# olivier-2018/scene_3Dreconstruction_MVSNet

Measured on AMD Instinct MI355X. Metric: depth maps/sec at N=5 views, 640x512, D=192; achieved HBM GB/s, higher is better.
Workload: dtype f32 (conv0, conv2-4, conv9, conv11: 3xbf16 split operands on the bf16 matrix cores, fp32 accumulate)

## Files before the change

scene_3dreconstruction_mvsnet_amd/csrc/conv0_split.hip:

```cpp
#include <cstdlib>
#include <cstring>
#include <type_traits>

#include "mvs_internal.h"
#include "storage.h"

#ifndef MVS_ABLATE
#define MVS_ABLATE 0
#endif

namespace mvs {

namespace c43s {
constexpr int TZ = 4, TY = 4, TX = 32;
constexpr int HY = TY + 2, HX = TX + 2;
constexpr int NT_PLANES = 6;
constexpr int VOX = HY * HX;
constexpr int PLANE_E = VOX * 8;
constexpr int PIECE_E = NT_PLANES * PLANE_E;
constexpr int TILE_E = 3 * PIECE_E;
constexpr int NCOL = VOX * 2;
constexpr int CPT = (NCOL + 255) / 256;
constexpr int NPOS = TY * TX;
constexpr int EXS = 12;
constexpr int BFRAG = 4 * NT_PLANES * 3 * 3;
static_assert(NT_PLANES * NPOS * EXS * 4 <= TILE_E * 2, "exchange tile must fit in the input tile");
}

typedef unsigned int su32x4 __attribute__((ext_vector_type(4)));
typedef unsigned int su32x2 __attribute__((ext_vector_type(2)));
typedef __bf16 sbf16x8 __attribute__((ext_vector_type(8)));
typedef __bf16 sbf16x4 __attribute__((ext_vector_type(4)));

__device__ __forceinline__ void split3(const f32x4 v, su32x2& p1, su32x2& p2, su32x2& p3) {
    const sbf16x4 h1 = __builtin_convertvector(v, sbf16x4);
    const f32x4 r1 = v - __builtin_convertvector(h1, f32x4);
    const sbf16x4 h2 = __builtin_convertvector(r1, sbf16x4);
    const f32x4 r2 = r1 - __builtin_convertvector(h2, f32x4);
    const sbf16x4 h3 = __builtin_convertvector(r2, sbf16x4);
    p1 = __builtin_bit_cast(su32x2, h1);
    p2 = __builtin_bit_cast(su32x2, h2);
    p3 = __builtin_bit_cast(su32x2, h3);
}

__device__ __forceinline__ f32x4 mfma_bf16(su32x4 a, su32x4 b, f32x4 c) {
    return __builtin_amdgcn_mfma_f32_16x16x32_bf16(__builtin_bit_cast(sbf16x8, a), __builtin_bit_cast(sbf16x8, b), c, 0, 0, 0);
}

template <int PAR>
__device__ __forceinline__ void c43s_chunk_mfmas(const unsigned short* __restrict__ tile, const int (&aoff)[3],
                                                 const su32x4 (&B)[2][3][3], f32x4 (&acc)[3][2]) {
    using namespace c43s;
#pragma unroll
    for (int p = 0; p < 3; ++p) {
        su32x4 a[3][4];
#pragma unroll
        for (int i = 0; i < 3; ++i)
#pragma unroll
            for (int j = 0; j < 4; ++j)
                a[i][j] = *reinterpret_cast<const su32x4*>(tile + p * PIECE_E + aoff[i] + j * HX * 8);
#pragma unroll
        for (int ky = 0; ky < 3; ++ky)
#pragma unroll
            for (int q = 0; q < 3 - p; ++q)
#pragma unroll
                for (int i = 0; i < 3; ++i) {
                    const int pl = i == 0 ? 0 : (i == 2 ? 1 : PAR);
#pragma unroll
                    for (int rr = 0; rr < 2; ++rr)
                        acc[i][rr] = mfma_bf16(a[i][rr + ky], B[pl][ky][q], acc[i][rr]);
                }
    }
}

__global__ __launch_bounds__(256, 2) void conv0_w43s_kernel(
    const float* __restrict__ x,
    const unsigned short* __restrict__ bp,
    const float* __restrict__ bias,
    float* __restrict__ y,
    int D, int H, int W
#if MVS_ABLATE == 50
    , long long* __restrict__ dbg
#endif
    ) {
    using namespace c43s;
#if MVS_ABLATE == 50
#define MVS_TICK(slot) if (dbg && blockIdx.x == 2000 && (threadIdx.x & 63) == 0) dbg[(threadIdx.x >> 6) * 32 + (slot)] = clock64();
#else
#define MVS_TICK(slot)
#endif
    __shared__ __attribute__((aligned(16))) unsigned short tile[TILE_E];

    const int tid = threadIdx.x, lane = tid & 63, wave = tid >> 6;
    const int nbx = (W + TX - 1) / TX, nby = (H + TY - 1) / TY;
    int bx, by, bz;
    if (nby % 8 == 0 && gridDim.x % 8 == 0) {
        const int xcd = blockIdx.x & 7, rows = nby >> 3;
        int i = blockIdx.x >> 3;
        bx = i % nbx; i /= nbx;
        by = xcd * rows + i % rows;
        bz = i / rows;
    } else {
        int b = blockIdx.x;
        bx = b % nbx; b /= nbx;
        by = b % nby;
        bz = b / nby;
    }
    const int x0 = bx * TX, y0 = by * TY, z0 = bz * TZ;
    const size_t HW8 = (size_t)H * W * 8, V8 = (size_t)D * HW8;

    unsigned boff[CPT][NT_PLANES];
    int loff[CPT];
#pragma unroll
    for (int i = 0; i < CPT; ++i) {
        const int col = tid + i * 256;
        const int half = col & 1, v = col >> 1;
        const int hx = v % HX, hy = v / HX;
        const int gy = y0 + hy - 1, gx = x0 + hx - 1;
        const bool ok = col < NCOL && gy >= 0 && gy < H && gx >= 0 && gx < W;
        loff[i] = col < NCOL ? v * 2 + half : -1;
#pragma unroll
        for (int q = 0; q < NT_PLANES; ++q) {
            const int gz = z0 - 1 + q;
            boff[i][q] = (ok && gz >= 0 && gz < D) ? (unsigned)(((size_t)gz * HW8 + ((size_t)gy * W + gx) * 8 + half * 4) * 4)
                                                   : 0x80000000u;
        }
    }
    f32x4 stg[CPT][NT_PLANES];
    auto load_chunk = [&](int c) {
        const __amdgpu_buffer_rsrc_t rs = __builtin_amdgcn_make_buffer_rsrc(
            const_cast<float*>(x + (size_t)c * V8), (short)0, (int)(V8 * 4), 0x00020000);
#pragma unroll
        for (int i = 0; i < CPT; ++i)
#pragma unroll
            for (int q = 0; q < NT_PLANES; ++q)
                stg[i][q] = __builtin_bit_cast(f32x4, __builtin_amdgcn_raw_buffer_load_b128(rs, (int)boff[i][q], 0, 0));
    };
    auto store_chunk = [&]() {
        su32x2* t8 = reinterpret_cast<su32x2*>(tile);
#pragma unroll
        for (int i = 0; i < CPT; ++i)
            if (loff[i] >= 0) {
                const f32x4(&d)[NT_PLANES] = stg[i];
                const f32x4 t1 = d[4] - 4.0f * d[2], t2 = d[3] - 4.0f * d[1];
                const f32x4 t3 = d[4] - d[2], t4 = 2.0f * (d[3] - d[1]);
                f32x4 u[NT_PLANES];
                u[0] = 4.0f * d[0] - 5.0f * d[2] + d[4];
                u[1] = t1 + t2;
                u[2] = t1 - t2;
                u[3] = t3 + t4;
                u[4] = t3 - t4;
                u[5] = 4.0f * d[1] - 5.0f * d[3] + d[5];
#pragma unroll
                for (int t = 0; t < NT_PLANES; ++t) {
                    su32x2 p1, p2, p3;
                    split3(u[t], p1, p2, p3);
                    su32x2* dst = t8 + t * (PLANE_E / 4) + loff[i];
                    dst[0] = p1;
                    dst[PIECE_E / 4] = p2;
                    dst[2 * (PIECE_E / 4)] = p3;
                }
            }
    };

    const int r = lane & 15, g = lane >> 4;
    const int u0 = 3 * wave, pA = u0 >> 1;
    int aoff[3];
#pragma unroll
    for (int i = 0; i < 3; ++i) {
        const int u = u0 + i, pl = u >> 1, mg = u & 1;
        aoff[i] = pl * PLANE_E + ((2 * mg) * HX + 2 * r + g) * 8;
    }
    su32x4 B[2][3][3];
    auto load_b = [&](int c) {
        const su32x4* bsrc = reinterpret_cast<const su32x4*>(bp) + (size_t)((c * NT_PLANES + pA) * 9) * 64 + lane;
#pragma unroll
        for (int pl = 0; pl < 2; ++pl)
#pragma unroll
            for (int ky = 0; ky < 3; ++ky)
#pragma unroll
                for (int q = 0; q < 3; ++q) B[pl][ky][q] = bsrc[((pl * 3 + ky) * 3 + q) * 64];
    };

    f32x4 acc[3][2];
#pragma unroll
    for (int i = 0; i < 3; ++i)
#pragma unroll
        for (int n = 0; n < 2; ++n) acc[i][n] = (f32x4){0.f, 0.f, 0.f, 0.f};

    MVS_TICK(0)
    load_chunk(0);
    load_b(0);
    store_chunk();
    MVS_TICK(1)
    __syncthreads();
    MVS_TICK(2)

#pragma unroll 1
    for (int c = 0; c < 4; ++c) {
        if (c < 3) load_chunk(c + 1);
        MVS_TICK(3 + 5 * c)
        if (wave & 1) c43s_chunk_mfmas<1>(tile, aoff, B, acc);
        else c43s_chunk_mfmas<0>(tile, aoff, B, acc);
        MVS_TICK(4 + 5 * c)
        if (c < 3) {
            load_b(c + 1);
            __syncthreads();
            MVS_TICK(5 + 5 * c)
            store_chunk();
            MVS_TICK(6 + 5 * c)
            __syncthreads();
            MVS_TICK(7 + 5 * c)
        }
    }

    __syncthreads();
    float* ex = reinterpret_cast<float*>(tile);
    {
        const int n = lane & 15, jj = n >> 3, co = n & 7;
#pragma unroll
        for (int i = 0; i < 3; ++i) {
            const int u = u0 + i, pl = u >> 1, mg = u & 1;
#pragma unroll
            for (int rr = 0; rr < 2; ++rr)
#pragma unroll
                for (int e = 0; e < 4; ++e)
                    ex[(pl * NPOS + (2 * mg + rr) * TX + 2 * (4 * g + e) + jj) * EXS + co] = acc[i][rr][e];
        }
    }
    __syncthreads();
    const int pos = tid >> 1, ch = tid & 1;
    const int gy = y0 + (pos >> 5), gx = x0 + (pos & 31);
    if (gy >= H || gx >= W) return;
    f32x4 M[NT_PLANES];
#pragma unroll
    for (int q = 0; q < NT_PLANES; ++q) M[q] = *reinterpret_cast<const f32x4*>(ex + (q * NPOS + pos) * EXS + ch * 4);
    const f32x4 bv = *reinterpret_cast<const f32x4*>(bias + ch * 4);
    const f32x4 zero = (f32x4){0.f, 0.f, 0.f, 0.f};
    const f32x4 s12 = M[1] + M[2], d12 = M[1] - M[2], s34 = M[3] + M[4], d34 = M[3] - M[4];
    f32x4 o[TZ];
    o[0] = (M[0] + s12) + s34;
    o[1] = d12 + 2.0f * d34;
    o[2] = s12 + 4.0f * s34;
    o[3] = (d12 + 8.0f * d34) + M[5];
#pragma unroll
    for (int q = 0; q < TZ; ++q) {
        if (z0 + q >= D) break;
        const f32x4 v = __builtin_elementwise_max(o[q] + bv, zero);
        *reinterpret_cast<f32x4*>(y + (((size_t)(z0 + q) * H + gy) * W + gx) * 8 + ch * 4) = v;
    }
    MVS_TICK(24)
#undef MVS_TICK
}

constexpr int c43p_MAXT = 512;
typedef float sf32x2 __attribute__((ext_vector_type(2)));
typedef __bf16 sbf16x2 __attribute__((ext_vector_type(2)));

__device__ __forceinline__ sf32x2 split_stage(const sf32x2 a, unsigned& packed) {
    const sbf16x2 h = __builtin_convertvector(a, sbf16x2);
    packed = __builtin_bit_cast(unsigned, h);
    const sf32x2 w = {__uint_as_float(packed << 16), __uint_as_float(packed & 0xFFFF0000u)};
    return a - w;
}
__device__ __forceinline__ void split3x(const f32x4 v, su32x2& p1, su32x2& p2, su32x2& p3) {
    unsigned a0, a1, b0, b1, c0, c1;
    const sf32x2 r0 = split_stage((sf32x2){v.x, v.y}, a0), r1 = split_stage((sf32x2){v.z, v.w}, a1);
    const sf32x2 q0 = split_stage(r0, b0), q1 = split_stage(r1, b1);
    c0 = __builtin_bit_cast(unsigned, __builtin_convertvector(q0, sbf16x2));
    c1 = __builtin_bit_cast(unsigned, __builtin_convertvector(q1, sbf16x2));
    p1 = (su32x2){a0, a1};
    p2 = (su32x2){b0, b1};
    p3 = (su32x2){c0, c1};
}

template <int PAR>
__device__ __forceinline__ void c43p_step_mfmas(const unsigned short* __restrict__ tile, const int (&aoff)[3],
                                                const su32x4 (&B)[2][3][3], su32x4 (&Bn)[2][3][3],
                                                __amdgpu_buffer_rsrc_t brs, unsigned bvoff, unsigned bnext,
                                                f32x4 (&acc)[3][2]) {
    using namespace c43s;
    constexpr int NC = 9;
    su32x4 a[3][4];
    auto request = [&](int n) {
        const int pn = n / 3, in = n % 3;
#pragma unroll
        for (int j = 0; j < 4; ++j)
            a[n % 3][j] = *reinterpret_cast<const su32x4*>(tile + pn * PIECE_E + aoff[in] + j * HX * 8);
    };
    request(0);
    request(1);
#pragma unroll
    for (int n = 0; n < NC; ++n) {
        const int p = n / 3, i = n % 3;
        if (n + 2 < NC) request(n + 2);
        {
            const int f0 = 2 * n, f1 = 2 * n + 1;
            Bn[f0 / 9][(f0 / 3) % 3][f0 % 3] = __builtin_bit_cast(su32x4, __builtin_amdgcn_raw_buffer_load_b128(
                brs, (int)bvoff, (int)(bnext + (unsigned)f0 * 1024u), 0));
            Bn[f1 / 9][(f1 / 3) % 3][f1 % 3] = __builtin_bit_cast(su32x4, __builtin_amdgcn_raw_buffer_load_b128(
                brs, (int)bvoff, (int)(bnext + (unsigned)f1 * 1024u), 0));
        }
        const int pl = i == 0 ? 0 : (i == 2 ? 1 : PAR);
#pragma unroll
        for (int ky = 0; ky < 3; ++ky)
#pragma unroll
            for (int q = 0; q < 3 - p; ++q)
#pragma unroll
                for (int rr = 0; rr < 2; ++rr)
                    acc[i][rr] = mfma_bf16(a[n % 3][rr + ky], B[pl][ky][q], acc[i][rr]);
#if MVS_ABLATE != 58
        __builtin_amdgcn_sched_barrier(0);
#endif
    }
}

__global__ __launch_bounds__(512) void conv0_w43p_kernel(
    const float* __restrict__ x,
    const unsigned short* __restrict__ bp,
    const float* __restrict__ bias,
    float* __restrict__ y,
    int D, int H, int W, int nb
#if MVS_ABLATE == 55
    , long long* __restrict__ dbg
#endif
    ) {
    using namespace c43s;
#if MVS_ABLATE == 55
#define MVS_PTICK(k, slot) if (dbg && blockIdx.x == 100 && (k) == 5 && (threadIdx.x & 63) == 0 && ((threadIdx.x >> 6) & 3) == 0) dbg[(threadIdx.x >> 8) * 64 + (slot)] = clock64();
#else
#define MVS_PTICK(k, slot)
#endif
    __shared__ __attribute__((aligned(16))) unsigned short buf[2 * TILE_E];
    __shared__ __attribute__((aligned(16))) float ex[NT_PLANES * NPOS * EXS];
    __shared__ int org[c43p_MAXT][4];

#if MVS_ABLATE == 75
    const int lane = threadIdx.x & 63, pw_ = threadIdx.x >> 6;
    const int wave = ((pw_ & 2) << 1) | ((pw_ & 4) >> 1) | (pw_ & 1), tid = wave * 64 + lane;
#else
    const int tid = threadIdx.x, lane = tid & 63, wave = tid >> 6;
#endif
    const bool consumer = __builtin_amdgcn_readfirstlane(wave) < 4;
    const int nbx = (W + TX - 1) / TX, nby = (H + TY - 1) / TY;
    const int G = gridDim.x;
    const int ntile = (nb - (int)blockIdx.x + G - 1) / G;
    const size_t HW8 = (size_t)H * W * 8, V8 = (size_t)D * HW8;
    auto origin = [&](int idx, int& x0, int& y0, int& z0) {
        int bx, by, bz;
        if (nby % 8 == 0 && G % 8 == 0) {
            const int xcd = idx & 7, rows = nby >> 3;
            int i = idx >> 3;
            bx = i % nbx; i /= nbx;
            by = xcd * rows + i % rows;
            bz = i / rows;
        } else {
            int b = idx;
            bx = b % nbx; b /= nbx;
            by = b % nby;
            bz = b / nby;
        }
        x0 = bx * TX; y0 = by * TY; z0 = bz * TZ;
    };

    for (int j = tid; j < ntile; j += 512) {
        int x0, y0, z0;
        origin((int)blockIdx.x + j * G, x0, y0, z0);
        org[j][0] = x0; org[j][1] = y0; org[j][2] = z0;
    }
    __syncthreads();
    const int ptid = tid & 255;
    unsigned boff[CPT][NT_PLANES];
    int loff[CPT];
    int chy[CPT], chx[CPT], crel[CPT];
#pragma unroll
    for (int i = 0; i < CPT; ++i) {
        const int col = min(ptid + i * 256, NCOL - 1);
        loff[i] = col;
        const int half = col & 1, v = col >> 1;
        chx[i] = v % HX - 1;
        chy[i] = v / HX - 1;
        crel[i] = (chy[i] * W + chx[i]) * 8 + half * 4;
    }
    auto set_tile = [&](int j) {
        const int x0 = org[j][0], y0 = org[j][1], z0 = org[j][2];
        const int hw8 = (int)HW8, tbase = (y0 * W + x0) * 8;
#pragma unroll
        for (int i = 0; i < CPT; ++i) {
            const int gy = y0 + chy[i], gx = x0 + chx[i];
            const bool ok = (unsigned)gy < (unsigned)H && (unsigned)gx < (unsigned)W;
            const int cb = tbase + crel[i];
#pragma unroll
            for (int q = 0; q < NT_PLANES; ++q) {
                const int gz = z0 - 1 + q;
                boff[i][q] = (ok && (unsigned)gz < (unsigned)D) ? (unsigned)(gz * hw8 + cb) * 4u
                                                                  : 0x80000000u;
            }
        }
    };
    f32x4 stg[2][CPT][NT_PLANES];
    auto issue_loads = [&](int c, f32x4 (&st)[CPT][NT_PLANES]) {
        const __amdgpu_buffer_rsrc_t rs = __builtin_amdgcn_make_buffer_rsrc(
            const_cast<float*>(x + (size_t)c * V8), (short)0, (int)(V8 * 4), 0x00020000);
#pragma unroll
        for (int i = 0; i < CPT; ++i)
#pragma unroll
            for (int q = 0; q < NT_PLANES; ++q)
                st[i][q] = __builtin_bit_cast(f32x4, __builtin_amdgcn_raw_buffer_load_b128(rs, (int)boff[i][q], 0, 0));
    };
    auto process = [&](auto set_tag, unsigned short* dstbuf, auto load_tag, int cn) {
        constexpr int SET = decltype(set_tag)::value;
        constexpr bool LOAD = decltype(load_tag)::value;
        su32x2* t8 = reinterpret_cast<su32x2*>(dstbuf);
        const __amdgpu_buffer_rsrc_t rs = __builtin_amdgcn_make_buffer_rsrc(
            const_cast<float*>(x + (size_t)cn * V8), (short)0, (int)(V8 * 4), 0x00020000);
#pragma unroll
        for (int i = 0; i < CPT; ++i) {
            f32x4 d[NT_PLANES];
#pragma unroll
            for (int q = 0; q < NT_PLANES; ++q) d[q] = stg[SET][i][q];
            const f32x4 t1 = d[4] - 4.0f * d[2], t2 = d[3] - 4.0f * d[1];
            const f32x4 t3 = d[4] - d[2], t4 = 2.0f * (d[3] - d[1]);
            f32x4 u[NT_PLANES];
            u[0] = 4.0f * d[0] - 5.0f * d[2] + d[4];
            u[1] = t1 + t2;
            u[2] = t1 - t2;
            u[3] = t3 + t4;
            u[4] = t3 - t4;
            u[5] = 4.0f * d[1] - 5.0f * d[3] + d[5];
#pragma unroll
            for (int t = 0; t < NT_PLANES; ++t) {
                if constexpr (LOAD)
                    stg[SET ^ 1][i][t] = __builtin_bit_cast(f32x4, __builtin_amdgcn_raw_buffer_load_b128(rs, (int)boff[i][t], 0, 0));
                su32x2 p1, p2, p3;
#if MVS_ABLATE == 74
                p1 = p2 = p3 = (su32x2){__float_as_uint(u[t].x), __float_as_uint(u[t].z)};
#else
                split3x(u[t], p1, p2, p3);
#endif
                su32x2* dst = t8 + t * (PLANE_E / 4) + loff[i];
                dst[0] = p1;
                dst[PIECE_E / 4] = p2;
                dst[2 * (PIECE_E / 4)] = p3;
#if MVS_ABLATE != 56
                __builtin_amdgcn_sched_barrier(0);
#endif
            }
        }
    };
    const f32x4 obias = *reinterpret_cast<const f32x4*>(bias + (ptid & 1) * 4);
    const __amdgpu_buffer_rsrc_t yrs = __builtin_amdgcn_make_buffer_rsrc(y, (short)0, (int)(V8 * 4), 0x00020000);
    auto output = [&](int j, bool live) {
        const int x0 = org[j][0], y0 = org[j][1], z0 = org[j][2];
        const int pos = ptid >> 1, ch = ptid & 1;
        const int gy = y0 + (pos >> 5), gx = x0 + (pos & 31);
        const bool ok = live && gy < H && gx < W;
        f32x4 M[NT_PLANES];
#pragma unroll
        for (int q = 0; q < NT_PLANES; ++q) M[q] = *reinterpret_cast<const f32x4*>(ex + (q * NPOS + pos) * EXS + ch * 4);
        const f32x4 zero = (f32x4){0.f, 0.f, 0.f, 0.f};
        const f32x4 s12 = M[1] + M[2], d12 = M[1] - M[2], s34 = M[3] + M[4], d34 = M[3] - M[4];
        f32x4 o[TZ];
        o[0] = (M[0] + s12) + s34;
        o[1] = d12 + 2.0f * d34;
        o[2] = s12 + 4.0f * s34;
        o[3] = (d12 + 8.0f * d34) + M[5];
        const unsigned base = (unsigned)((((size_t)z0 * H + gy) * W + gx) * 8 + ch * 4) * 4u;
#pragma unroll
        for (int q = 0; q < TZ; ++q) {
            const f32x4 v = __builtin_elementwise_max(o[q] + obias, zero);
            const unsigned off = (ok && z0 + q < D) ? base + (unsigned)q * (unsigned)(HW8 * 4) : 0xFFFFFFF0u;
            __builtin_amdgcn_raw_buffer_store_b128(__builtin_bit_cast(su32x4, v), yrs, (int)off, 0, 0);
        }
    };

    const int r = lane & 15, g = lane >> 4;
    const int cw = wave & 3, u0 = 3 * cw, pA = u0 >> 1;
    int aoff[3];
#pragma unroll
    for (int i = 0; i < 3; ++i) {
        const int u = u0 + i, pl = u >> 1, mg = u & 1;
        aoff[i] = pl * PLANE_E + ((2 * mg) * HX + 2 * r + g) * 8;
    }
    su32x4 B[2][2][3][3];
    const __amdgpu_buffer_rsrc_t brs = __builtin_amdgcn_make_buffer_rsrc(
        const_cast<unsigned short*>(bp), (short)0, 4 * NT_PLANES * 9 * 1024, 0x00020000);
    const unsigned bvoff = (unsigned)lane * 16u + (unsigned)pA * 9u * 1024u;
    auto load_b = [&](int c, su32x4 (&Bd)[2][3][3]) {
#pragma unroll
        for (int pl = 0; pl < 2; ++pl)
#pragma unroll
            for (int ky = 0; ky < 3; ++ky)
#pragma unroll
                for (int q = 0; q < 3; ++q)
                    Bd[pl][ky][q] = __builtin_bit_cast(su32x4, __builtin_amdgcn_raw_buffer_load_b128(
                        brs, (int)bvoff, (int)((unsigned)((c * NT_PLANES * 3 + pl * 3 + ky) * 3 + q) * 1024u), 0));
    };
    f32x4 acc[3][2];
#pragma unroll
    for (int i = 0; i < 3; ++i)
#pragma unroll
        for (int n = 0; n < 2; ++n) acc[i][n] = (f32x4){0.f, 0.f, 0.f, 0.f};
    auto exchange = [&]() {
        const int n = lane & 15, jj = n >> 3, co = n & 7;
#pragma unroll
        for (int i = 0; i < 3; ++i) {
            const int u = u0 + i, pl = u >> 1, mg = u & 1;
#pragma unroll
            for (int rr = 0; rr < 2; ++rr)
#pragma unroll
                for (int e = 0; e < 4; ++e) {
                    ex[(pl * NPOS + (2 * mg + rr) * TX + 2 * (4 * g + e) + jj) * EXS + co] = acc[i][rr][e];
                    acc[i][rr][e] = 0.0f;
                }
        }
    };

    if (consumer) {
        int kk = 0;
        auto cstep = [&](auto c_tag) {
            constexpr int c = decltype(c_tag)::value, PB = c & 1;
            MVS_PTICK(kk, 4 * c + 0)
            if (c == 1) output(kk > 0 ? kk - 1 : 0, kk > 0);
            constexpr unsigned bnext = (unsigned)(((c + 1) & 3) * NT_PLANES * 9) * 1024u;
            MVS_PTICK(kk, 4 * c + 1)
#if MVS_ABLATE == 71
            if (D < 0)
#endif
            {
            if (cw & 1) c43p_step_mfmas<1>(buf + PB * TILE_E, aoff, B[PB], B[PB ^ 1], brs, bvoff, bnext, acc);
            else c43p_step_mfmas<0>(buf + PB * TILE_E, aoff, B[PB], B[PB ^ 1], brs, bvoff, bnext, acc);
            }
            MVS_PTICK(kk, 4 * c + 2)
            if (c == 3) exchange();
            MVS_PTICK(kk, 4 * c + 3)
        };
        load_b(0, B[0]);
        __syncthreads();
#pragma unroll 1
        for (int k = 0; k < ntile; ++k) {
            kk = k;
            cstep(std::integral_constant<int, 0>{});
            __syncthreads();
            cstep(std::integral_constant<int, 1>{});
            __syncthreads();
            cstep(std::integral_constant<int, 2>{});
            __syncthreads();
            cstep(std::integral_constant<int, 3>{});
            __syncthreads();
            MVS_PTICK(k, 16)
        }
        output(ntile - 1, true);
    } else {
#if MVS_ABLATE != 57
        __builtin_amdgcn_s_setprio(2);
#endif
        auto pstep = [&](int k, auto c_tag) {
            constexpr int c = decltype(c_tag)::value, PB = c & 1;
            MVS_PTICK(k, 4 * c + 0)
            if (c == 2 && k + 1 < ntile) set_tile(k + 1);
            MVS_PTICK(k, 4 * c + 1)
            MVS_PTICK(k, 4 * c + 2)
            process(std::integral_constant<int, PB ^ 1>{}, buf + (PB ^ 1) * TILE_E, std::true_type{}, (c + 2) & 3);
            MVS_PTICK(k, 4 * c + 3)
        };
        set_tile(0);
        issue_loads(0, stg[0]);
        issue_loads(1, stg[1]);
        process(std::integral_constant<int, 0>{}, buf, std::false_type{}, 0);
        __syncthreads();
#pragma unroll 1
        for (int k = 0; k < ntile; ++k) {
            pstep(k, std::integral_constant<int, 0>{});
            __syncthreads();
            pstep(k, std::integral_constant<int, 1>{});
            __syncthreads();
            pstep(k, std::integral_constant<int, 2>{});
            __syncthreads();
            pstep(k, std::integral_constant<int, 3>{});
            __syncthreads();
            MVS_PTICK(k, 16)
        }
    }
}

int launch_conv0_wino43_split(const void* x, void* y, const void* bp, const float* bias, int D, int H, int W,
                              int dtype, hipStream_t s) {
    using namespace c43s;
    if (dtype != MVS_F32) return fail(MVS_ERR_BAD_DTYPE, "conv0_wino43_split: fp32 volumes only (dtype %d)", dtype);
    if ((size_t)D * H * W * 8 * 4 >= ((size_t)1 << 31))
        return fail(MVS_ERR_BAD_SHAPE, "conv0_wino43_split: plane of %zu bytes exceeds 31-bit buffer offsets",
                    (size_t)D * H * W * 8 * 4);
    const int nb = ((W + TX - 1) / TX) * ((H + TY - 1) / TY) * ((D + TZ - 1) / TZ);
    static const bool form1 = [] {
        const char* e = getenv("MVS_CONV0_SPLIT");
        return e && e[0] == '2';
    }();

    if (!form1) {
        int dev = 0, cus = 256;
        if (hipGetDevice(&dev) != hipSuccess ||
            hipDeviceGetAttribute(&cus, hipDeviceAttributeMultiprocessorCount, dev) != hipSuccess)
            cus = 256;
        int grid = nb < cus ? nb : cus;
        if ((nb + grid - 1) / grid > c43p_MAXT) grid = (nb + c43p_MAXT - 1) / c43p_MAXT;
#if MVS_ABLATE == 55
        static long long* dbgp = nullptr;
        if (!dbgp && hipMalloc(&dbgp, 128 * sizeof(long long)) != hipSuccess) dbgp = nullptr;
        if (dbgp) (void)hipMemsetAsync(dbgp, 0, 128 * sizeof(long long), s);
        conv0_w43p_kernel<<<grid, 512, 0, s>>>(static_cast<const float*>(x), static_cast<const unsigned short*>(bp), bias,
                                               static_cast<float*>(y), D, H, W, nb, dbgp);
        if (dbgp && grid > 100) {
            long long h[128];
            (void)hipStreamSynchronize(s);
            (void)hipMemcpy(h, dbgp, sizeof(h), hipMemcpyDeviceToHost);
            for (int role = 0; role < 2; ++role) {
                const long long* t = h + role * 64;
                fprintf(stderr, "conv0p %s:", role ? "producer (loads | output | process | barrier)" : "consumer (B loads | mfma | exchange | barrier)");
                for (int c = 0; c < 4; ++c)
                    fprintf(stderr, " c%d: %lld %lld %lld %lld |", c, t[4 * c + 1] - t[4 * c], t[4 * c + 2] - t[4 * c + 1],
                            t[4 * c + 3] - t[4 * c + 2], (c < 3 ? t[4 * c + 4] : t[16]) - t[4 * c + 3]);
                fprintf(stderr, " tile %lld\n", t[16] - t[0]);
            }
        }
#else
        conv0_w43p_kernel<<<grid, 512, 0, s>>>(static_cast<const float*>(x), static_cast<const unsigned short*>(bp), bias,
                                               static_cast<float*>(y), D, H, W, nb);
#endif
        return check_hip(hipGetLastError(), "conv0_w43p launch");
    }
#if MVS_ABLATE == 50
    static long long* dbg = nullptr;
    if (!dbg && hipMalloc(&dbg, 128 * sizeof(long long)) != hipSuccess) dbg = nullptr;
    if (dbg) (void)hipMemsetAsync(dbg, 0, 128 * sizeof(long long), s);
    conv0_w43s_kernel<<<nb, 256, 0, s>>>(static_cast<const float*>(x), static_cast<const unsigned short*>(bp), bias,
                                         static_cast<float*>(y), D, H, W, dbg);
    if (dbg && nb > 2000) {
        long long h[128];
        (void)hipStreamSynchronize(s);
        (void)hipMemcpy(h, dbg, sizeof(h), hipMemcpyDeviceToHost);
        for (int w = 0; w < 4; ++w) {
            const long long* t = h + w * 32;
            fprintf(stderr, "conv0s wave %d: stage0 %lld bar %lld |", w, t[1] - t[0], t[2] - t[1]);
            for (int c = 0; c < 4; ++c)
                fprintf(stderr, " c%d: ld %lld mfma %lld bar %lld st %lld bar %lld |", c, t[3 + 5 * c] - (c ? t[2 + 5 * c] : t[2]),
                        t[4 + 5 * c] - t[3 + 5 * c], c < 3 ? t[5 + 5 * c] - t[4 + 5 * c] : 0, c < 3 ? t[6 + 5 * c] - t[5 + 5 * c] : 0,
                        c < 3 ? t[7 + 5 * c] - t[6 + 5 * c] : 0);
            fprintf(stderr, " end %lld total %lld\n", t[24] - t[19], t[24] - t[0]);
        }
    }
#else
    conv0_w43s_kernel<<<nb, 256, 0, s>>>(static_cast<const float*>(x), static_cast<const unsigned short*>(bp), bias,
                                         static_cast<float*>(y), D, H, W);
#endif
    return check_hip(hipGetLastError(), "conv0_w43s launch");
}

static inline uint16_t bf16_rne(float v) {
    uint32_t u;
    std::memcpy(&u, &v, 4);
    if ((u & 0x7F800000u) == 0x7F800000u && (u & 0x007FFFFFu)) return (uint16_t)((u >> 16) | 0x0040u);
    u += 0x7FFFu + ((u >> 16) & 1u);
    return (uint16_t)(u >> 16);
}
static inline float bf16_to_f32(uint16_t h) {
    const uint32_t u = (uint32_t)h << 16;
    float v;
    std::memcpy(&v, &u, 4);
    return v;
}

void pack_conv0_wino43_split_weights(const float* wfold, void* out) {
    uint16_t* bp = static_cast<uint16_t*>(out);
    for (int c = 0; c < 4; ++c)
        for (int t = 0; t < 6; ++t)
            for (int ky = 0; ky < 3; ++ky)
                for (int lane = 0; lane < 64; ++lane)
                    for (int j = 0; j < 8; ++j) {
                        const int n = lane & 15, g = lane >> 4, jj = n >> 3, co = n & 7, kx = g - jj;
                        float gv = 0.0f;
                        if (kx >= 0 && kx <= 2) {
                            const int tap = ky * 3 + kx, ci = 8 * c + j;
                            const double g0 = wfold[((size_t)(0 * 9 + tap) * 32 + ci) * 8 + co];
                            const double g1 = wfold[((size_t)(1 * 9 + tap) * 32 + ci) * 8 + co];
                            const double g2 = wfold[((size_t)(2 * 9 + tap) * 32 + ci) * 8 + co];
                            double gd;
                            switch (t) {
                                case 0: gd = g0 / 4.0; break;
                                case 1: gd = -(g0 + g1 + g2) / 6.0; break;
                                case 2: gd = -(g0 - g1 + g2) / 6.0; break;
                                case 3: gd = g0 / 24.0 + g1 / 12.0 + g2 / 6.0; break;
                                case 4: gd = g0 / 24.0 - g1 / 12.0 + g2 / 6.0; break;
                                default: gd = g2; break;
                            }
                            gv = (float)gd;
                        }
                        const uint16_t h1 = bf16_rne(gv);
                        const float r1 = gv - bf16_to_f32(h1);
                        const uint16_t h2 = bf16_rne(r1);
                        const float r2 = r1 - bf16_to_f32(h2);
                        const uint16_t h3 = bf16_rne(r2);
                        const uint16_t hs[3] = {h1, h2, h3};
                        for (int q = 0; q < 3; ++q)
                            bp[((((size_t)(c * 6 + t) * 3 + ky) * 3 + q) * 64 + lane) * 8 + j] = hs[q];
                    }
}

}
```

Measured before the change: 1463.

## Enlarge conv0 Winograd tile to 4x8x32 with half-plane producer/consumer pipeline

Replaces the default conv0 split-bf16 Winograd kernel with a variant whose spatial tile is 8 rows instead of 4. Each tile's six transformed planes are now staged in two halves of three planes across eight barrier-separated steps. Consumers keep two sets of accumulators and interleave output between steps. The producer defers half of the transformed planes in registers, and the load chunk order zigzags between tiles so the next B fragments can be reused. The aim is to cut halo overhead and per-tile B-weight reloads, at the cost of more register pressure, more barriers, and LDS close to its limit. The CU count query is also cached per device.

```diff
diff --git a/scene_3dreconstruction_mvsnet_amd/csrc/conv0_split.hip b/scene_3dreconstruction_mvsnet_amd/csrc/conv0_split.hip
--- a/scene_3dreconstruction_mvsnet_amd/csrc/conv0_split.hip
+++ b/scene_3dreconstruction_mvsnet_amd/csrc/conv0_split.hip
@@ -1,3 +1,4 @@
+#include <atomic>
 #include <cstdlib>
 #include <cstring>
 #include <type_traits>
@@ -23,7 +24,6 @@
 constexpr int CPT = (NCOL + 255) / 256;
 constexpr int NPOS = TY * TX;
 constexpr int EXS = 12;
-constexpr int BFRAG = 4 * NT_PLANES * 3 * 3;
 static_assert(NT_PLANES * NPOS * EXS * 4 <= TILE_E * 2, "exchange tile must fit in the input tile");
 }
 
@@ -253,7 +253,24 @@
 #undef MVS_TICK
 }
 
-constexpr int c43p_MAXT = 512;
+namespace c48t {
+constexpr int TZ = 4, TY = 8, TX = 32;
+constexpr int HY = TY + 2, HX = TX + 2;
+constexpr int NT_PLANES = 6, NPL = 3;
+constexpr int VOX = HY * HX;
+constexpr int PLANE_E = VOX * 8;
+constexpr int PIECE_E = NPL * PLANE_E;
+constexpr int BUF_E = 3 * PIECE_E;
+constexpr int NCOL = VOX * 2;
+constexpr int CPT = (NCOL + 255) / 256;
+constexpr int NPOS = TY * TX;
+constexpr int EXS = 8;
+constexpr int MAXT = 512;
+static_assert(2 * BUF_E * 2 + NT_PLANES * NPOS * EXS * 4 + MAXT * 16 <= 160 * 1024, "LDS of conv0_w48t");
+constexpr unsigned bstep(int s) { return (unsigned)(((s >> 1) * NT_PLANES + 3 * (s & 1)) * 9) * 1024u; }
+__device__ __forceinline__ int chunk_of(int k, int c) { return (k & 1) ? 3 - c : c; }
+__device__ __forceinline__ unsigned bofs(int chunk, int h) { return (unsigned)((chunk * NT_PLANES + 3 * h) * 9) * 1024u; }
+}
 typedef float sf32x2 __attribute__((ext_vector_type(2)));
 typedef __bf16 sbf16x2 __attribute__((ext_vector_type(2)));
 
@@ -274,12 +291,11 @@
     p3 = (su32x2){c0, c1};
 }
 
-template <int PAR>
-__device__ __forceinline__ void c43p_step_mfmas(const unsigned short* __restrict__ tile, const int (&aoff)[3],
+__device__ __forceinline__ void c48t_step_mfmas(const unsigned short* __restrict__ tile, const int (&aoff)[3],
                                                 const su32x4 (&B)[2][3][3], su32x4 (&Bn)[2][3][3],
-                                                __amdgpu_buffer_rsrc_t brs, unsigned bvoff, unsigned bnext,
+                                                __amdgpu_buffer_rsrc_t brs, const unsigned (&bvoff)[2], unsigned bnext,
                                                 f32x4 (&acc)[3][2]) {
-    using namespace c43s;
+    using namespace c48t;
     constexpr int NC = 9;
     su32x4 a[3][4];
     auto request = [&](int n) {
@@ -294,14 +310,11 @@
     for (int n = 0; n < NC; ++n) {
         const int p = n / 3, i = n % 3;
         if (n + 2 < NC) request(n + 2);
-        {
-            const int f0 = 2 * n, f1 = 2 * n + 1;
-            Bn[f0 / 9][(f0 / 3) % 3][f0 % 3] = __builtin_bit_cast(su32x4, __builtin_amdgcn_raw_buffer_load_b128(
-                brs, (int)bvoff, (int)(bnext + (unsigned)f0 * 1024u), 0));
-            Bn[f1 / 9][(f1 / 3) % 3][f1 % 3] = __builtin_bit_cast(su32x4, __builtin_amdgcn_raw_buffer_load_b128(
-                brs, (int)bvoff, (int)(bnext + (unsigned)f1 * 1024u), 0));
-        }
-        const int pl = i == 0 ? 0 : (i == 2 ? 1 : PAR);
+#pragma unroll
+        for (int f = 2 * n; f < 2 * n + 2; ++f)
+            Bn[f / 9][(f / 3) % 3][f % 3] = __builtin_bit_cast(su32x4, __builtin_amdgcn_raw_buffer_load_b128(
+                brs, (int)bvoff[f / 9], (int)(bnext + (unsigned)(f % 9) * 1024u), 0));
+        const int pl = i == 2 ? 1 : 0;
 #pragma unroll
         for (int ky = 0; ky < 3; ++ky)
 #pragma unroll
@@ -309,13 +322,11 @@
 #pragma unroll
                 for (int rr = 0; rr < 2; ++rr)
                     acc[i][rr] = mfma_bf16(a[n % 3][rr + ky], B[pl][ky][q], acc[i][rr]);
-#if MVS_ABLATE != 58
         __builtin_amdgcn_sched_barrier(0);
-#endif
-    }
-}
-
-__global__ __launch_bounds__(512) void conv0_w43p_kernel(
+    }
+}
+
+__global__ __launch_bounds__(512) void conv0_w48t_kernel(
     const float* __restrict__ x,
     const unsigned short* __restrict__ bp,
     const float* __restrict__ bias,
@@ -325,22 +336,17 @@
     , long long* __restrict__ dbg
 #endif
     ) {
-    using namespace c43s;
+    using namespace c48t;
 #if MVS_ABLATE == 55
 #define MVS_PTICK(k, slot) if (dbg && blockIdx.x == 100 && (k) == 5 && (threadIdx.x & 63) == 0 && ((threadIdx.x >> 6) & 3) == 0) dbg[(threadIdx.x >> 8) * 64 + (slot)] = clock64();
 #else
 #define MVS_PTICK(k, slot)
 #endif
-    __shared__ __attribute__((aligned(16))) unsigned short buf[2 * TILE_E];
+    __shared__ __attribute__((aligned(16))) unsigned short buf[2 * BUF_E];
     __shared__ __attribute__((aligned(16))) float ex[NT_PLANES * NPOS * EXS];
-    __shared__ int org[c43p_MAXT][4];
-
-#if MVS_ABLATE == 75
-    const int lane = threadIdx.x & 63, pw_ = threadIdx.x >> 6;
-    const int wave = ((pw_ & 2) << 1) | ((pw_ & 4) >> 1) | (pw_ & 1), tid = wave * 64 + lane;
-#else
+    __shared__ int org[MAXT][4];
+
     const int tid = threadIdx.x, lane = tid & 63, wave = tid >> 6;
-#endif
     const bool consumer = __builtin_amdgcn_readfirstlane(wave) < 4;
     const int nbx = (W + TX - 1) / TX, nby = (H + TY - 1) / TY;
     const int G = gridDim.x;
@@ -370,172 +376,85 @@
     }
     __syncthreads();
     const int ptid = tid & 255;
-    unsigned boff[CPT][NT_PLANES];
-    int loff[CPT];
-    int chy[CPT], chx[CPT], crel[CPT];
-#pragma unroll
-    for (int i = 0; i < CPT; ++i) {
-        const int col = min(ptid + i * 256, NCOL - 1);
-        loff[i] = col;
-        const int half = col & 1, v = col >> 1;
-        chx[i] = v % HX - 1;
-        chy[i] = v / HX - 1;
-        crel[i] = (chy[i] * W + chx[i]) * 8 + half * 4;
-    }
-    auto set_tile = [&](int j) {
-        const int x0 = org[j][0], y0 = org[j][1], z0 = org[j][2];
-        const int hw8 = (int)HW8, tbase = (y0 * W + x0) * 8;
-#pragma unroll
-        for (int i = 0; i < CPT; ++i) {
-            const int gy = y0 + chy[i], gx = x0 + chx[i];
-            const bool ok = (unsigned)gy < (unsigned)H && (unsigned)gx < (unsigned)W;
-            const int cb = tbase + crel[i];
-#pragma unroll
-            for (int q = 0; q < NT_PLANES; ++q) {
-                const int gz = z0 - 1 + q;
-                boff[i][q] = (ok && (unsigned)gz < (unsigned)D) ? (unsigned)(gz * hw8 + cb) * 4u
-                                                                  : 0x80000000u;
+
+    if (consumer) {
+        const int r = lane & 15, g = lane >> 4, cw = wave;
+        const int pa = (0x2100 >> (4 * cw)) & 15, ra = (0x1220 >> (4 * cw)) & 15;
+        const int pb = (0x2211 >> (4 * cw)) & 15, rb = (0x3010 >> (4 * cw)) & 15;
+        const int upl[3] = {pa, pa, pb}, urp[3] = {ra, ra + 1, rb};
+        int aoff[3];
+#pragma unroll
+        for (int i = 0; i < 3; ++i) aoff[i] = upl[i] * PLANE_E + ((2 * urp[i]) * HX + 2 * r + g) * 8;
+        su32x4 B[2][2][3][3];
+        const __amdgpu_buffer_rsrc_t brs = __builtin_amdgcn_make_buffer_rsrc(
+            const_cast<unsigned short*>(bp), (short)0, 4 * NT_PLANES * 9 * 1024, 0x00020000);
+        const unsigned bvoff[2] = {(unsigned)lane * 16u + (unsigned)pa * 9u * 1024u,
+                                   (unsigned)lane * 16u + (unsigned)pb * 9u * 1024u};
+#pragma unroll
+        for (int f = 0; f < 18; ++f)
+            B[0][f / 9][(f / 3) % 3][f % 3] = __builtin_bit_cast(su32x4, __builtin_amdgcn_raw_buffer_load_b128(
+                brs, (int)bvoff[f / 9], (int)(bstep(0) + (unsigned)(f % 9) * 1024u), 0));
+        f32x4 acc[2][3][2];
+#pragma unroll
+        for (int h = 0; h < 2; ++h)
+#pragma unroll
+            for (int i = 0; i < 3; ++i)
+#pragma unroll
+                for (int n = 0; n < 2; ++n) acc[h][i][n] = (f32x4){0.f, 0.f, 0.f, 0.f};
+        auto exchange = [&]() {
+            const int n = lane & 15, jj = n >> 3, co = n & 7;
+#pragma unroll
+            for (int h = 0; h < 2; ++h)
+#pragma unroll
+                for (int i = 0; i < 3; ++i)
+#pragma unroll
+                    for (int rr = 0; rr < 2; ++rr)
+#pragma unroll
+                        for (int e = 0; e < 4; ++e) {
+                            ex[((3 * h + upl[i]) * NPOS + (2 * urp[i] + rr) * TX + 2 * (4 * g + e) + jj) * EXS + co] = acc[h][i][rr][e];
+                            acc[h][i][rr][e] = 0.0f;
+                        }
+        };
+        const __amdgpu_buffer_rsrc_t yrs = __builtin_amdgcn_make_buffer_rsrc(y, (short)0, (int)(V8 * 4), 0x00020000);
+        const f32x4 obias = *reinterpret_cast<const f32x4*>(bias + (ptid & 1) * 4);
+        auto output = [&](int j, int it, bool live) {
+            const int x0 = org[j][0], y0 = org[j][1], z0 = org[j][2];
+            const int pos = (ptid >> 1) + it * (NPOS / 2), ch = ptid & 1;
+            const int gy = y0 + (pos >> 5), gx = x0 + (pos & 31);
+            const bool ok = live && gy < H && gx < W;
+            f32x4 M[NT_PLANES];
+#pragma unroll
+            for (int q = 0; q < NT_PLANES; ++q) M[q] = *reinterpret_cast<const f32x4*>(ex + (q * NPOS + pos) * EXS + ch * 4);
+            const f32x4 zero = (f32x4){0.f, 0.f, 0.f, 0.f};
+            const f32x4 s12 = M[1] + M[2], d12 = M[1] - M[2], s34 = M[3] + M[4], d34 = M[3] - M[4];
+            f32x4 o[TZ];
+            o[0] = (M[0] + s12) + s34;
+            o[1] = d12 + 2.0f * d34;
+            o[2] = s12 + 4.0f * s34;
+            o[3] = (d12 + 8.0f * d34) + M[5];
+            const unsigned base = (unsigned)((((size_t)z0 * H + gy) * W + gx) * 8 + ch * 4) * 4u;
+#pragma unroll
+            for (int q = 0; q < TZ; ++q) {
+                const f32x4 v = __builtin_elementwise_max(o[q] + obias, zero);
+                const unsigned off = (ok && z0 + q < D) ? base + (unsigned)q * (unsigned)(HW8 * 4) : 0xFFFFFFF0u;
+                __builtin_amdgcn_raw_buffer_store_b128(__builtin_bit_cast(su32x4, v), yrs, (int)off, 0, 0);
             }
-        }
-    };
-    f32x4 stg[2][CPT][NT_PLANES];
-    auto issue_loads = [&](int c, f32x4 (&st)[CPT][NT_PLANES]) {
-        const __amdgpu_buffer_rsrc_t rs = __builtin_amdgcn_make_buffer_rsrc(
-            const_cast<float*>(x + (size_t)c * V8), (short)0, (int)(V8 * 4), 0x00020000);
-#pragma unroll
-        for (int i = 0; i < CPT; ++i)
-#pragma unroll
-            for (int q = 0; q < NT_PLANES; ++q)
-                st[i][q] = __builtin_bit_cast(f32x4, __builtin_amdgcn_raw_buffer_load_b128(rs, (int)boff[i][q], 0, 0));
-    };
-    auto process = [&](auto set_tag, unsigned short* dstbuf, auto load_tag, int cn) {
-        constexpr int SET = decltype(set_tag)::value;
-        constexpr bool LOAD = decltype(load_tag)::value;
-        su32x2* t8 = reinterpret_cast<su32x2*>(dstbuf);
-        const __amdgpu_buffer_rsrc_t rs = __builtin_amdgcn_make_buffer_rsrc(
-            const_cast<float*>(x + (size_t)cn * V8), (short)0, (int)(V8 * 4), 0x00020000);
-#pragma unroll
-        for (int i = 0; i < CPT; ++i) {
-            f32x4 d[NT_PLANES];
-#pragma unroll
-            for (int q = 0; q < NT_PLANES; ++q) d[q] = stg[SET][i][q];
-            const f32x4 t1 = d[4] - 4.0f * d[2], t2 = d[3] - 4.0f * d[1];
-            const f32x4 t3 = d[4] - d[2], t4 = 2.0f * (d[3] - d[1]);
-            f32x4 u[NT_PLANES];
-            u[0] = 4.0f * d[0] - 5.0f * d[2] + d[4];
-            u[1] = t1 + t2;
-            u[2] = t1 - t2;
-            u[3] = t3 + t4;
-            u[4] = t3 - t4;
-            u[5] = 4.0f * d[1] - 5.0f * d[3] + d[5];
-#pragma unroll
-            for (int t = 0; t < NT_PLANES; ++t) {
-                if constexpr (LOAD)
-                    stg[SET ^ 1][i][t] = __builtin_bit_cast(f32x4, __builtin_amdgcn_raw_buffer_load_b128(rs, (int)boff[i][t], 0, 0));
-                su32x2 p1, p2, p3;
-#if MVS_ABLATE == 74
-                p1 = p2 = p3 = (su32x2){__float_as_uint(u[t].x), __float_as_uint(u[t].z)};
-#else
-                split3x(u[t], p1, p2, p3);
-#endif
-                su32x2* dst = t8 + t * (PLANE_E / 4) + loff[i];
-                dst[0] = p1;
-                dst[PIECE_E / 4] = p2;
-                dst[2 * (PIECE_E / 4)] = p3;
-#if MVS_ABLATE != 56
-                __builtin_amdgcn_sched_barrier(0);
-#endif
-            }
-        }
-    };
-    const f32x4 obias = *reinterpret_cast<const f32x4*>(bias + (ptid & 1) * 4);
-    const __amdgpu_buffer_rsrc_t yrs = __builtin_amdgcn_make_buffer_rsrc(y, (short)0, (int)(V8 * 4), 0x00020000);
-    auto output = [&](int j, bool live) {
-        const int x0 = org[j][0], y0 = org[j][1], z0 = org[j][2];
-        const int pos = ptid >> 1, ch = ptid & 1;
-        const int gy = y0 + (pos >> 5), gx = x0 + (pos & 31);
-        const bool ok = live && gy < H && gx < W;
-        f32x4 M[NT_PLANES];
-#pragma unroll
-        for (int q = 0; q < NT_PLANES; ++q) M[q] = *reinterpret_cast<const f32x4*>(ex + (q * NPOS + pos) * EXS + ch * 4);
-        const f32x4 zero = (f32x4){0.f, 0.f, 0.f, 0.f};
-        const f32x4 s12 = M[1] + M[2], d12 = M[1] - M[2], s34 = M[3] + M[4], d34 = M[3] - M[4];
-        f32x4 o[TZ];
-        o[0] = (M[0] + s12) + s34;
-        o[1] = d12 + 2.0f * d34;
-        o[2] = s12 + 4.0f * s34;
-        o[3] = (d12 + 8.0f * d34) + M[5];
-        const unsigned base = (unsigned)((((size_t)z0 * H + gy) * W + gx) * 8 + ch * 4) * 4u;
-#pragma unroll
-        for (int q = 0; q < TZ; ++q) {
-            const f32x4 v = __builtin_elementwise_max(o[q] + obias, zero);
-            const unsigned off = (ok && z0 + q < D) ? base + (unsigned)q * (unsigned)(HW8 * 4) : 0xFFFFFFF0u;
-            __builtin_amdgcn_raw_buffer_store_b128(__builtin_bit_cast(su32x4, v), yrs, (int)off, 0, 0);
-        }
-    };
-
-    const int r = lane & 15, g = lane >> 4;
-    const int cw = wave & 3, u0 = 3 * cw, pA = u0 >> 1;
-    int aoff[3];
-#pragma unroll
-    for (int i = 0; i < 3; ++i) {
-        const int u = u0 + i, pl = u >> 1, mg = u & 1;
-        aoff[i] = pl * PLANE_E + ((2 * mg) * HX + 2 * r + g) * 8;
-    }
-    su32x4 B[2][2][3][3];
-    const __amdgpu_buffer_rsrc_t brs = __builtin_amdgcn_make_buffer_rsrc(
-        const_cast<unsigned short*>(bp), (short)0, 4 * NT_PLANES * 9 * 1024, 0x00020000);
-    const unsigned bvoff = (unsigned)lane * 16u + (unsigned)pA * 9u * 1024u;
-    auto load_b = [&](int c, su32x4 (&Bd)[2][3][3]) {
-#pragma unroll
-        for (int pl = 0; pl < 2; ++pl)
-#pragma unroll
-            for (int ky = 0; ky < 3; ++ky)
-#pragma unroll
-                for (int q = 0; q < 3; ++q)
-                    Bd[pl][ky][q] = __builtin_bit_cast(su32x4, __builtin_amdgcn_raw_buffer_load_b128(
-                        brs, (int)bvoff, (int)((unsigned)((c * NT_PLANES * 3 + pl * 3 + ky) * 3 + q) * 1024u), 0));
-    };
-    f32x4 acc[3][2];
-#pragma unroll
-    for (int i = 0; i < 3; ++i)
-#pragma unroll
-        for (int n = 0; n < 2; ++n) acc[i][n] = (f32x4){0.f, 0.f, 0.f, 0.f};
-    auto exchange = [&]() {
-        const int n = lane & 15, jj = n >> 3, co = n & 7;
-#pragma unroll
-        for (int i = 0; i < 3; ++i) {
-            const int u = u0 + i, pl = u >> 1, mg = u & 1;
-#pragma unroll
-            for (int rr = 0; rr < 2; ++rr)
-#pragma unroll
-                for (int e = 0; e < 4; ++e) {
-                    ex[(pl * NPOS + (2 * mg + rr) * TX + 2 * (4 * g + e) + jj) * EXS + co] = acc[i][rr][e];
-                    acc[i][rr][e] = 0.0f;
-                }
-        }
-    };
-
-    if (consumer) {
+        };
         int kk = 0;
-        auto cstep = [&](auto c_tag) {
-            constexpr int c = decltype(c_tag)::value, PB = c & 1;
-            MVS_PTICK(kk, 4 * c + 0)
-            if (c == 1) output(kk > 0 ? kk - 1 : 0, kk > 0);
-            constexpr unsigned bnext = (unsigned)(((c + 1) & 3) * NT_PLANES * 9) * 1024u;
-            MVS_PTICK(kk, 4 * c + 1)
+        auto cstep = [&](auto s_tag) {
+            constexpr int s = decltype(s_tag)::value, h = s & 1;
+            MVS_PTICK(kk, 4 * s + 0)
+            if (s == 1 || s == 3) output(kk > 0 ? kk - 1 : 0, s >> 1, kk > 0);
+            MVS_PTICK(kk, 4 * s + 1)
 #if MVS_ABLATE == 71
             if (D < 0)
 #endif
-            {
-            if (cw & 1) c43p_step_mfmas<1>(buf + PB * TILE_E, aoff, B[PB], B[PB ^ 1], brs, bvoff, bnext, acc);
-            else c43p_step_mfmas<0>(buf + PB * TILE_E, aoff, B[PB], B[PB ^ 1], brs, bvoff, bnext, acc);
-            }
-            MVS_PTICK(kk, 4 * c + 2)
-            if (c == 3) exchange();
-            MVS_PTICK(kk, 4 * c + 3)
-        };
-        load_b(0, B[0]);
+            c48t_step_mfmas(buf + h * BUF_E, aoff, B[h], B[h ^ 1], brs, bvoff,
+                            s < 7 ? bofs(chunk_of(kk, (s + 1) >> 1), (s + 1) & 1) : bofs(chunk_of(kk + 1, 0), 0), acc[h]);
+            MVS_PTICK(kk, 4 * s + 2)
+            if (s == 7) exchange();
+            MVS_PTICK(kk, 4 * s + 3)
+        };
         __syncthreads();
 #pragma unroll 1
         for (int k = 0; k < ntile; ++k) {
@@ -548,26 +467,117 @@
             __syncthreads();
             cstep(std::integral_constant<int, 3>{});
             __syncthreads();
-            MVS_PTICK(k, 16)
-        }
-        output(ntile - 1, true);
+            cstep(std::integral_constant<int, 4>{});
+            __syncthreads();
+            cstep(std::integral_constant<int, 5>{});
+            __syncthreads();
+            cstep(std::integral_constant<int, 6>{});
+            __syncthreads();
+            cstep(std::integral_constant<int, 7>{});
+            __syncthreads();
+            MVS_PTICK(k, 32)
+        }
+        output(ntile - 1, 0, true);
+        output(ntile - 1, 1, true);
     } else {
 #if MVS_ABLATE != 57
         __builtin_amdgcn_s_setprio(2);
 #endif
-        auto pstep = [&](int k, auto c_tag) {
-            constexpr int c = decltype(c_tag)::value, PB = c & 1;
-            MVS_PTICK(k, 4 * c + 0)
-            if (c == 2 && k + 1 < ntile) set_tile(k + 1);
-            MVS_PTICK(k, 4 * c + 1)
-            MVS_PTICK(k, 4 * c + 2)
-            process(std::integral_constant<int, PB ^ 1>{}, buf + (PB ^ 1) * TILE_E, std::true_type{}, (c + 2) & 3);
-            MVS_PTICK(k, 4 * c + 3)
+        unsigned boff[CPT][NT_PLANES];
+        int loff[CPT];
+        int chy[CPT], chx[CPT], crel[CPT];
+#pragma unroll
+        for (int i = 0; i < CPT; ++i) {
+            const int col = min(ptid + i * 256, NCOL - 1);
+            loff[i] = col;
+            const int half = col & 1, v = col >> 1;
+            chx[i] = v % HX - 1;
+            chy[i] = v / HX - 1;
+            crel[i] = (chy[i] * W + chx[i]) * 8 + half * 4;
+        }
+        auto set_tile = [&](int j) {
+            const int x0 = org[j][0], y0 = org[j][1], z0 = org[j][2];
+            const int hw8 = (int)HW8, tbase = (y0 * W + x0) * 8;
+#pragma unroll
+            for (int i = 0; i < CPT; ++i) {
+                const int gy = y0 + chy[i], gx = x0 + chx[i];
+                const bool ok = (unsigned)gy < (unsigned)H && (unsigned)gx < (unsigned)W;
+                const int cb = tbase + crel[i];
+#pragma unroll
+                for (int q = 0; q < NT_PLANES; ++q) {
+                    const int gz = z0 - 1 + q;
+                    boff[i][q] = (ok && (unsigned)gz < (unsigned)D) ? (unsigned)(gz * hw8 + cb) * 4u
+                                                                      : 0x80000000u;
+                }
+            }
+        };
+        auto rsrc = [&](int c) {
+            return __builtin_amdgcn_make_buffer_rsrc(const_cast<float*>(x + (size_t)c * V8), (short)0, (int)(V8 * 4), 0x00020000);
+        };
+        f32x4 stg[CPT][NT_PLANES];
+        f32x4 hold[CPT][NPL];
+        auto put = [&](unsigned short* dstbuf, int i, int t, const f32x4 u) {
+            su32x2 p1, p2, p3;
+            split3x(u, p1, p2, p3);
+            su32x2* dst = reinterpret_cast<su32x2*>(dstbuf) + t * (PLANE_E / 4) + loff[i];
+            dst[0] = p1;
+            dst[PIECE_E / 4] = p2;
+            dst[2 * (PIECE_E / 4)] = p3;
+        };
+        auto process0 = [&](int cn) {
+            const __amdgpu_buffer_rsrc_t rs = rsrc(cn);
+#pragma unroll
+            for (int i = 0; i < CPT; ++i) {
+                f32x4 d[NT_PLANES];
+#pragma unroll
+                for (int q = 0; q < NT_PLANES; ++q) d[q] = stg[i][q];
+                const f32x4 t1 = d[4] - 4.0f * d[2], t2 = d[3] - 4.0f * d[1];
+                const f32x4 t3 = d[4] - d[2], t4 = 2.0f * (d[3] - d[1]);
+                const f32x4 u0 = 4.0f * d[0] - 5.0f * d[2] + d[4];
+                const f32x4 u1 = t1 + t2, u2 = t1 - t2;
+                hold[i][0] = t3 + t4;
+                hold[i][1] = t3 - t4;
+                hold[i][2] = 4.0f * d[1] - 5.0f * d[3] + d[5];
+                const f32x4 u[NPL] = {u0, u1, u2};
+#pragma unroll
+                for (int t = 0; t < NPL; ++t) {
+#pragma unroll
+                    for (int q = 2 * t; q < 2 * t + 2; ++q)
+                        stg[i][q] = __builtin_bit_cast(f32x4, __builtin_amdgcn_raw_buffer_load_b128(rs, (int)boff[i][q], 0, 0));
+                    put(buf, i, t, u[t]);
+                    __builtin_amdgcn_sched_barrier(0);
+                }
+            }
+        };
+        auto process1 = [&]() {
+#pragma unroll
+            for (int i = 0; i < CPT; ++i)
+#pragma unroll
+                for (int t = 0; t < NPL; ++t) {
+                    put(buf + BUF_E, i, t, hold[i][t]);
+                    __builtin_amdgcn_sched_barrier(0);
+                }
+        };
+        auto pstep = [&](int k, auto s_tag) {
+            constexpr int s = decltype(s_tag)::value, c = s >> 1, h = s & 1;
+            MVS_PTICK(k, 4 * s + 0)
+            if (s == 5 && k + 1 < ntile) set_tile(k + 1);
+            MVS_PTICK(k, 4 * s + 1)
+            MVS_PTICK(k, 4 * s + 2)
+            if (h == 0) process1();
+            else process0(c < 2 ? chunk_of(k, c + 2) : chunk_of(k + 1, c - 2));
+            MVS_PTICK(k, 4 * s + 3)
         };
         set_tile(0);
-        issue_loads(0, stg[0]);
-        issue_loads(1, stg[1]);
-        process(std::integral_constant<int, 0>{}, buf, std::false_type{}, 0);
+        {
+            const __amdgpu_buffer_rsrc_t rs = rsrc(0);
+#pragma unroll
+            for (int i = 0; i < CPT; ++i)
+#pragma unroll
+                for (int q = 0; q < NT_PLANES; ++q)
+                    stg[i][q] = __builtin_bit_cast(f32x4, __builtin_amdgcn_raw_buffer_load_b128(rs, (int)boff[i][q], 0, 0));
+        }
+        process0(1);
         __syncthreads();
 #pragma unroll 1
         for (int k = 0; k < ntile; ++k) {
@@ -579,36 +589,54 @@
             __syncthreads();
             pstep(k, std::integral_constant<int, 3>{});
             __syncthreads();
-            MVS_PTICK(k, 16)
-        }
-    }
+            pstep(k, std::integral_constant<int, 4>{});
+            __syncthreads();
+            pstep(k, std::integral_constant<int, 5>{});
+            __syncthreads();
+            pstep(k, std::integral_constant<int, 6>{});
+            __syncthreads();
+            pstep(k, std::integral_constant<int, 7>{});
+            __syncthreads();
+            MVS_PTICK(k, 32)
+        }
+    }
+#undef MVS_PTICK
+}
+
+static int device_cus() {
+    static std::atomic<int> cache[64];
+    int dev = 0;
+    if (hipGetDevice(&dev) != hipSuccess || dev < 0 || dev >= 64) return 256;
+    int n = cache[dev].load(std::memory_order_relaxed);
+    if (n == 0) {
+        if (hipDeviceGetAttribute(&n, hipDeviceAttributeMultiprocessorCount, dev) != hipSuccess || n <= 0) n = 256;
+        cache[dev].store(n, std::memory_order_relaxed);
+    }
+    return n;
 }
 
 int launch_conv0_wino43_split(const void* x, void* y, const void* bp, const float* bias, int D, int H, int W,
                               int dtype, hipStream_t s) {
-    using namespace c43s;
     if (dtype != MVS_F32) return fail(MVS_ERR_BAD_DTYPE, "conv0_wino43_split: fp32 volumes only (dtype %d)", dtype);
     if ((size_t)D * H * W * 8 * 4 >= ((size_t)1 << 31))
         return fail(MVS_ERR_BAD_SHAPE, "conv0_wino43_split: plane of %zu bytes exceeds 31-bit buffer offsets",
                     (size_t)D * H * W * 8 * 4);
-    const int nb = ((W + TX - 1) / TX) * ((H + TY - 1) / TY) * ((D + TZ - 1) / TZ);
     static const bool form1 = [] {
         const char* e = getenv("MVS_CONV0_SPLIT");
         return e && e[0] == '2';
     }();
 
     if (!form1) {
-        int dev = 0, cus = 256;
-        if (hipGetDevice(&dev) != hipSuccess ||
-            hipDeviceGetAttribute(&cus, hipDeviceAttributeMultiprocessorCount, dev) != hipSuccess)
-            cus = 256;
+        using namespace c48t;
+        const int nb = ((W + TX - 1) / TX) * ((H + TY - 1) / TY) * ((D + TZ - 1) / TZ);
+        const int cus = device_cus();
         int grid = nb < cus ? nb : cus;
-        if ((nb + grid - 1) / grid > c43p_MAXT) grid = (nb + c43p_MAXT - 1) / c43p_MAXT;
+        if ((nb + grid - 1) / grid > MAXT) grid = (nb + MAXT - 1) / MAXT;
 #if MVS_ABLATE == 55
         static long long* dbgp = nullptr;
         if (!dbgp && hipMalloc(&dbgp, 128 * sizeof(long long)) != hipSuccess) dbgp = nullptr;
         if (dbgp) (void)hipMemsetAsync(dbgp, 0, 128 * sizeof(long long), s);
-        conv0_w43p_kernel<<<grid, 512, 0, s>>>(static_cast<const float*>(x), static_cast<const unsigned short*>(bp), bias,
+        conv0_w48t_kernel<<<grid, 512, 0, s>>>(static_cast<const float*>(x), static_cast<const unsigned short*>(bp), bias,
                                                static_cast<float*>(y), D, H, W, nb, dbgp);
         if (dbgp && grid > 100) {
             long long h[128];
@@ -616,19 +644,21 @@
             (void)hipMemcpy(h, dbgp, sizeof(h), hipMemcpyDeviceToHost);
             for (int role = 0; role < 2; ++role) {
                 const long long* t = h + role * 64;
-                fprintf(stderr, "conv0p %s:", role ? "producer (loads | output | process | barrier)" : "consumer (B loads | mfma | exchange | barrier)");
-                for (int c = 0; c < 4; ++c)
-                    fprintf(stderr, " c%d: %lld %lld %lld %lld |", c, t[4 * c + 1] - t[4 * c], t[4 * c + 2] - t[4 * c + 1],
-                            t[4 * c + 3] - t[4 * c + 2], (c < 3 ? t[4 * c + 4] : t[16]) - t[4 * c + 3]);
-                fprintf(stderr, " tile %lld\n", t[16] - t[0]);
+                fprintf(stderr, "conv0t %s:", role ? "producer (set_tile | - | process | barrier)" : "consumer (output | mfma | exchange | barrier)");
+                for (int c = 0; c < 8; ++c)
+                    fprintf(stderr, " s%d: %lld %lld %lld %lld |", c, t[4 * c + 1] - t[4 * c], t[4 * c + 2] - t[4 * c + 1],
+                            t[4 * c + 3] - t[4 * c + 2], t[4 * c + 4] - t[4 * c + 3]);
+                fprintf(stderr, " tile %lld\n", t[32] - t[0]);
             }
         }
 #else
-        conv0_w43p_kernel<<<grid, 512, 0, s>>>(static_cast<const float*>(x), static_cast<const unsigned short*>(bp), bias,
+        conv0_w48t_kernel<<<grid, 512, 0, s>>>(static_cast<const float*>(x), static_cast<const unsigned short*>(bp), bias,
                                                static_cast<float*>(y), D, H, W, nb);
 #endif
-        return check_hip(hipGetLastError(), "conv0_w43p launch");
-    }
+        return check_hip(hipGetLastError(), "conv0_w48t launch");
+    }
+    using namespace c43s;
+    const int nb = ((W + TX - 1) / TX) * ((H + TY - 1) / TY) * ((D + TZ - 1) / TZ);
 #if MVS_ABLATE == 50
     static long long* dbg = nullptr;
     if (!dbg && hipMalloc(&dbg, 128 * sizeof(long long)) != hipSuccess) dbg = nullptr;
```

Result: faster. 1509, median of 6 (+3.1%).
